# NethermindEth/latticefold

Hardware: AMD Instinct MI355X
Metric: folding-prover steps/sec (one NIFSProver::prove per step), GoldilocksRingNTT (higher is better)
Workload: dtype u64; 1 GPU; C4: GoldilocksRingNTT R1CS->CCS, m=N=2^20 rows, wit_len=262144, L=4, B=2^16, b=2, K=16, kappa=26, t=3; parallelism=replicas x1

## Files before the change

latticefold_amd/csrc/lf_capi.cpp:

```cpp
#include "lf_ring_host.h"
#include <thread>
#include <vector>

const char *lf_strerror(int code) {
    switch (code) {
        case LF_OK: return "ok";
        case LF_ERR_INVALID: return "invalid argument / wrong length";
        case LF_ERR_HIP: return "HIP runtime error (no GPU or out of device memory)";
        case LF_ERR_UNSUPPORTED: return "unsupported parameter";
        case LF_ERR_BAD_TABLES: return "ring tables are not a ring isomorphism";
        case LF_ERR_NORM: return "witness coefficient exceeds the decomposition bound";
        case LF_ERR_SIZE_BOUNDS: return "invalid size bounds (m must be >= wit_len*L, power of two)";
        case LF_ERR_STATE: return "call sequence misuse";
        case LF_ERR_REJECT: return "verifier rejected the proof";
    }
    return "unknown error";
}
const char *lf_phase_name(int i) { return (i >= 0 && i < LF_N_PHASES) ? PHASE_NAMES[i] : ""; }

static int install_tables(lf_ctx *c, u64 nonres, const u64 *y) {
    CrtTables T;
    if (build_crt_tables(nonres, y, T) != 0) return LF_ERR_BAD_TABLES;
    c->ring.T = T;
    c->dcrt = make_dev_crt(T);
    return ring_ops<GoldRing>::install_icrt(c, &T.icrt[0][0]);
}

int lf_ctx_create_ring(lf_ctx **out, int device, int ring) {
    if (ring == LF_RING_GOLDILOCKS) return lf_ctx_create(out, device);
    if (!out || ring != LF_RING_BABYBEAR) return LF_ERR_INVALID;
    lf_ctx *c = new lf_ctx();
    c->device = device;
    int rc = lfbb::BbCtx::create(&c->bb, c, device);
    if (rc != LF_OK) { delete c; return rc; }
    *out = c;
    return LF_OK;
}
int lf_ctx_device(const lf_ctx *c) { return c->device; }
int lf_ctx_ring(const lf_ctx *c) { return c && c->bb ? LF_RING_BABYBEAR : LF_RING_GOLDILOCKS; }
int lf_ring_words(int ring) { return ring == LF_RING_BABYBEAR ? 72 : (ring == LF_RING_GOLDILOCKS ? 24 : 0); }
int lf_ring_tau(int ring) { return ring == LF_RING_BABYBEAR ? 9 : (ring == LF_RING_GOLDILOCKS ? 3 : 0); }
uint64_t lf_ring_modulus(int ring) { return ring == LF_RING_BABYBEAR ? (uint64_t)lfbb::BB_P : (ring == LF_RING_GOLDILOCKS ? LF_P : 0); }

int lf_ctx_create(lf_ctx **out, int device) {
    if (!out) return LF_ERR_INVALID;
    int cnt = 0;
    if (hipGetDeviceCount(&cnt) != hipSuccess || cnt <= 0 || device < 0 || device >= cnt) return LF_ERR_HIP;
    HIPCHK(hipSetDevice(device));
    lf_ctx *c = new lf_ctx();
    c->device = device;
    int least = 0, greatest = 0;
    (void)hipDeviceGetStreamPriorityRange(&least, &greatest);
    if (c->create_lane_streams() != LF_OK || hipStreamCreateWithPriority(&c->st_io, hipStreamDefault, least) != hipSuccess) { delete c; return LF_ERR_HIP; }
    (void)hipEventCreateWithFlags(&c->ev_block, hipEventBlockingSync | hipEventDisableTiming);
    u64 nr, y[24];
    default_ring(&nr, y);
    int rc = install_tables(c, nr, y);
    if (rc != LF_OK) { delete c; return rc; }
    *out = c;
    return LF_OK;
}
static void planes_pool_drop(int device);
void lf_ctx_destroy(lf_ctx *c) {
    if (!c) return;
    while (c->io_jobs.load() > 0) std::this_thread::yield();
    (void)hipSetDevice(c->device);
    planes_pool_drop(c->device);
    if (c->bb) { c->bb->destroy(); delete c; return; }
    (void)c->sync_lanes();
    if (c->st_io) (void)hipStreamSynchronize(c->st_io);
    for (int l = 0; l < LF_NLANES; l++)
        if (c->stage[l]) (void)hipHostFree(c->stage[l]);
    if (c->h_pin2) { (void)hipHostFree(c->h_pin2); c->h_pin2 = nullptr; }
    if (c->ev_block) (void)hipEventDestroy(c->ev_block);
    c->comm[0].destroy();
    c->comm[1].destroy();
    if (c->tail_mail) (void)hipHostFree(c->tail_mail);
    if (c->tail_counters) (void)hipFree(c->tail_counters);
    if (c->d_poseidon) (void)hipFree(c->d_poseidon);
    if (c->ev_theta) (void)hipEventDestroy(c->ev_theta);
    if (c->ev_aux) (void)hipEventDestroy(c->ev_aux);
    if (c->st_aux) (void)hipStreamDestroy(c->st_aux);
    if (c->h_aux) (void)hipHostFree(c->h_aux);
    for (int i = 0; i < 2; i++)
        if (c->bits_ev[i]) (void)hipEventDestroy(c->bits_ev[i]);
    c->release_core();
    delete c;
}
int lf_set_ring_tables(lf_ctx *c, uint64_t nonres, const uint64_t *y) {
    if (!c || !y) return LF_ERR_INVALID;
    if (c->bb) return c->bb->set_ring_tables(nonres, y);
    std::lock_guard<std::mutex> g(c->mu);
    HIPCHK(hipSetDevice(c->device));
    return install_tables(c, nonres, y);
}
int lf_get_ring_tables(lf_ctx *c, uint64_t *nonres, uint64_t *y) {
    if (!c || !nonres || !y) return LF_ERR_INVALID;
    if (c->bb) return c->bb->get_ring_tables(nonres, y);
    *nonres = c->ring.T.nu;
    for (int k = 0; k < 8; k++)
        for (int q = 0; q < 3; q++) y[3 * k + q] = c->ring.T.y[k].c[q];
    return LF_OK;
}

int lf_set_digit_mode(lf_ctx *c, int mode) {
    if (!c || (mode != 0 && mode != 1)) return LF_ERR_INVALID;
    std::lock_guard<std::mutex> g(c->mu);
    c->core_any().digit_mode = mode;
    return LF_OK;
}
int lf_set_ext_basis(lf_ctx *c, const uint64_t *T) {
    if (!c || !T) return LF_ERR_INVALID;
    std::lock_guard<std::mutex> g(c->mu);
    const int ring = lf_ctx_ring(c);
    ExtBasis nb = c->xb;
    RET(nb.set(T, lf_ring_tau(ring), lf_ring_modulus(ring)));
    c->xb = nb;
    const int tt = nb.tau * nb.tau;
    if (c->bb) {
        lfbb::BbCtxImpl *b = c->bb->p;
        std::lock_guard<std::mutex> gb(b->mu);
        b->xb_on = nb.on;
        for (int i = 0; i < tt; i++) { b->xb_T[i] = lfbb::from_canon(nb.T[i]); b->xb_Ti[i] = lfbb::from_canon(nb.Ti[i]); }
    } else {
        c->xb_on = nb.on;
        for (int i = 0; i < tt; i++) { c->xb_T[i] = nb.T[i]; c->xb_Ti[i] = nb.Ti[i]; }
    }
    return LF_OK;
}
int lf_set_sharding(lf_ctx *c, int rank, int world, lf_exchange_fn cb, void *user) {
    if (!c || world < 1 || rank < 0 || rank >= world || (world & (world - 1)) != 0 || (world > 1 && !cb)) return LF_ERR_INVALID;
    if (c->bb) return c->bb->set_sharding(rank, world, cb, user);
// ... 983 lines not shown
```

latticefold_amd/csrc/lf_common.h:

```cpp
#pragma once
#include <hip/hip_runtime.h>

#include <stdlib.h>

#include <atomic>

#include "../../include/lfhip.h"

#define HIPCHK(x)                                    \
    do {                                             \
        hipError_t e__ = (x);                        \
        if (e__ != hipSuccess) return LF_ERR_HIP;    \
    } while (0)
#define RET(x)                      \
    do {                            \
        int rc__ = (x);             \
        if (rc__ != LF_OK) return rc__; \
    } while (0)

extern "C" void lfplus_scratch_trim(int device);
template <class T> static inline hipError_t lf_dev_malloc(T **p, size_t bytes) {
    hipError_t e = hipMalloc((void **)p, bytes);
    if (e != hipErrorOutOfMemory) return e;
    (void)hipGetLastError();
// ... 20 lines not shown
        bytes = want;
        return LF_OK;
    }
    void release() {
        if (p) (void)hipFree(p);
        p = nullptr;
        bytes = 0;
    }
};

inline uint64_t lf_next_witness_id() {
    static std::atomic<uint64_t> next{1};
    return next.fetch_add(1, std::memory_order_relaxed);
}
struct lf_witness {
    lf_ctx *ctx;
    int32_t *planes;
    size_t N;
    int device;
    size_t plane_bytes;
    uint64_t id = lf_next_witness_id();
    uint64_t *f_ntt = nullptr;
    size_t f_bytes = 0;
    uint64_t *w_ccs = nullptr;
    size_t w_bytes = 0;
};

int lf_planes_alloc(lf_ctx *ctx, size_t bytes, int32_t **out);
void lf_planes_release(lf_ctx *ctx, size_t bytes, int32_t *p);
int lf_ctx_device(const lf_ctx *ctx);


struct Tunables {
    bool lin_u_eval = false, fold_unfused = false, fold_no_lut = false, fold_tab_r1 = false, theta_eval = false, fold_no_r4tab = false, fold_no_r5tab = false;
    bool fold_rounds_no_split = false;
    bool fold_sv_no_split = false;
    bool lin_no_split = false;
    size_t lin_split_min = (size_t)1 << 17;
    bool no_live_rows = false;
    bool live_rows_low = false;
    size_t fold_split_min = 8192;
    bool force_exchange = false;
    bool device_transcript = false;
    bool shard_plain_rounds = false;
    int shard_two_lanes = -1;
    size_t shard_lin_min = 16384;
    size_t shard_fold_min = 2048;
    long i8_wgs = 0;
    bool lin_no_r1cs = false;
    bool lin_no_small = false;
    size_t dot_min = 4096;
    bool dot_valu = false;
    bool fold_witness_valu = false;
    bool fold_no_sv = false;
    size_t sv_min = 65536;
    int sv_rounds = 3;
    bool no_tail = false;
    size_t fuse_min = 16384, lut_min = (size_t)1 << 17, tab_min = 16384;
    size_t r5_min = 8192;
    size_t tail_n = 2048;
    static Tunables read(size_t lut_min_default) {
        Tunables t;
        t.lut_min = lut_min_default;
        const char *e;
        t.lin_u_eval = getenv("LF_LIN_U_EVAL") != nullptr;
        t.fold_unfused = getenv("LF_FOLD_UNFUSED") != nullptr;
        t.fold_no_lut = getenv("LF_FOLD_NO_LUT") != nullptr;
        t.fold_tab_r1 = getenv("LF_FOLD_TAB_R1") != nullptr;
        t.fold_no_r4tab = getenv("LF_FOLD_NO_R4TAB") != nullptr;
        t.fold_no_r5tab = getenv("LF_FOLD_NO_R5TAB") != nullptr;
        t.lin_no_split = getenv("LF_LIN_NO_SPLIT") != nullptr;
        t.fold_sv_no_split = getenv("LF_FOLD_SV_NO_SPLIT") != nullptr;
        t.no_live_rows = getenv("LF_NO_LIVE_ROWS") != nullptr;
        t.live_rows_low = getenv("LF_LIVE_ROWS_LOW") != nullptr;
        t.fold_rounds_no_split = getenv("LF_FOLD_ROUNDS_NO_SPLIT") != nullptr;
        if (const char *e = getenv("LF_LIN_SPLIT_MIN")) t.lin_split_min = (size_t)atoll(e);
        if (const char *e = getenv("LF_FOLD_SPLIT_MIN")) t.fold_split_min = (size_t)atoll(e);
        t.theta_eval = getenv("LF_THETA_EVAL") != nullptr;
        t.no_tail = getenv("LF_NO_TAIL") != nullptr;
        t.fold_no_sv = getenv("LF_FOLD_NO_SV") != nullptr;
        t.dot_valu = getenv("LF_DOT_VALU") != nullptr;
        t.fold_witness_valu = getenv("LF_FOLD_WITNESS_VALU") != nullptr;
        if ((e = getenv("LF_DOT_MIN"))) t.dot_min = (size_t)atoll(e);
        t.lin_no_small = getenv("LF_LIN_NO_SMALL") != nullptr;
        t.lin_no_r1cs = getenv("LF_LIN_NO_R1CS") != nullptr;
        if ((e = getenv("LF_FOLD_SV_MIN"))) t.sv_min = (size_t)atoll(e);
        if ((e = getenv("LF_FOLD_SV_ROUNDS"))) t.sv_rounds = atoi(e);
        if ((e = getenv("LF_I8_WGS"))) t.i8_wgs = atol(e);
        if ((e = getenv("LF_SHARD_TWO_LANES"))) t.shard_two_lanes = atoi(e) != 0;
        if ((e = getenv("LF_SHARD_LIN_MIN"))) t.shard_lin_min = (size_t)atoll(e);
        if ((e = getenv("LF_SHARD_FOLD_MIN"))) t.shard_fold_min = (size_t)atoll(e);
        t.shard_plain_rounds = getenv("LF_SHARD_PLAIN_ROUNDS") != nullptr;
        t.device_transcript = getenv("LF_DEVICE_TRANSCRIPT") != nullptr;
        t.force_exchange = getenv("LF_DIST_FORCE_EXCHANGE") != nullptr;
        if ((e = getenv("LF_FOLD_FUSE_MIN"))) t.fuse_min = (size_t)atoll(e);
        if ((e = getenv("LF_FOLD_LUT_MIN"))) t.lut_min = (size_t)atoll(e);
        if ((e = getenv("LF_FOLD_TAB_MIN"))) t.tab_min = (size_t)atoll(e);
        if ((e = getenv("LF_TAIL_N"))) t.tail_n = (size_t)atoll(e);
        if ((e = getenv("LF_FOLD_R5_MIN"))) t.r5_min = (size_t)atoll(e);
        return t;
    }
};

static inline int lf_validate_csr(unsigned t, size_t m, size_t n, const uint32_t *const *rowptr, const uint32_t *const *col,
                                  const uint64_t *const *val, int words, uint64_t modulus) {
    for (unsigned j = 0; j < t; j++) {
        if (!rowptr[j] || !col[j] || !val[j]) return LF_ERR_INVALID;
        if (rowptr[j][0] != 0) return LF_ERR_INVALID;
        for (size_t r = 0; r < m; r++)
            if (rowptr[j][r + 1] < rowptr[j][r]) return LF_ERR_INVALID;
        const size_t nnz = rowptr[j][m];
        for (size_t k = 0; k < nnz; k++)
            if (col[j][k] >= n) return LF_ERR_INVALID;
        for (size_t k = 0; k < nnz * (size_t)words; k++)
            if (val[j][k] >= modulus) return LF_ERR_INVALID;
    }
    return LF_OK;
}

struct ExtBasis {
    bool on = false;
    int tau = 0;
    uint64_t p = 0;
    uint64_t T[81], Ti[81];
    static uint64_t mulmod(uint64_t a, uint64_t b, uint64_t p) { return (uint64_t)(((unsigned __int128)a * b) % p); }
    void apply(const uint64_t *M, uint64_t *v) const {
        uint64_t o[9];
        for (int i = 0; i < tau; i++) {
            unsigned __int128 acc = 0;
            for (int j = 0; j < tau; j++) acc += (unsigned __int128)mulmod(M[i * tau + j], v[j], p);
            o[i] = (uint64_t)(acc % p);
        }
        for (int i = 0; i < tau; i++) v[i] = o[i];
    }
    void to_ext(uint64_t *v, size_t slots) const { if (on) for (size_t s = 0; s < slots; s++) apply(T, v + s * tau); }
// ... 34 lines not shown
```

latticefold_amd/csrc/lf_ctx.h:

```cpp
#pragma once
#include <hip/hip_runtime.h>
#include <assert.h>
#include <string.h>

#include <atomic>
#include <chrono>
#include <condition_variable>
#include <functional>
#include <future>
#include <thread>
#include <map>
#include <memory>
#include <mutex>
#include <set>
#include <string>
#include <vector>

#include "../../include/lfhip.h"
#include "bb_capi.h"
#include "lf_ctx_core.h"
#include "lf_common.h"
#include "lf_dist.h"
#include "lf_kernels.h"
#include "lf_live_rows.h"
// ... 74 lines not shown
        std::unique_lock<std::mutex> lk(m);
        for (;;) {
            cv.wait(lk, [&] { return has_job || stop; });
            if (stop) return;
            std::function<int()> j = std::move(job);
            has_job = false;
            lk.unlock();
            int r = j();
            lk.lock();
            rc = r;
            done = true;
            cv.notify_all();
        }
    }
    void submit(std::function<int()> j) {
        std::unique_lock<std::mutex> lk(m);
        if (!th.joinable()) th = std::thread([this] { loop(); });
        job = std::move(j);
        has_job = true;
        done = false;
        cv.notify_all();
    }
    int wait() {
        std::unique_lock<std::mutex> lk(m);
        cv.wait(lk, [&] { return done; });
        return rc;
    }
    ~LaneWorker() {
        {
            std::unique_lock<std::mutex> lk(m);
            stop = true;
            cv.notify_all();
        }
        if (th.joinable()) th.join();
    }
};

struct lf_ctx : CtxCore<u64> {
    lf_ctx() : CtxCore<u64>(8192, 2 * 9 * 24 * sizeof(u64)) {}
    int lane() const override { return t_lane; }
    lfbb::BbCtx *bb = nullptr;
    ExtBasis xb;
    hipStream_t &st_io = st_lane[2];
    std::mutex io_mu;
    std::atomic<int> io_jobs{0};
    inline CtxCoreBase &core_any();
    bool have_ccs_any() { return core_any().have_ccs; }
    const lf_params &params_any() { return core_any().P; }
    size_t n_any() { return core_any().n; }
    size_t m_any() { return core_any().m; }
    size_t N_any() { return core_any().N; }
    HostRing ring;
    DevCrt dcrt;
    LaneWorker lane1;
    int agreed_two_lanes = -1;
    bool two_lanes_ok = false;
    lfdist::Comm comm[2];
    lfdist::Comm &cm() { assert(t_lane < 2); return comm[t_lane]; }
    bool ccs_general = false;
    size_t live_rows = 0;
    lflive::Plan live_plan() const {
        if (tn.no_live_rows || sh_world > 1) return lflive::plan(m, m, 0, 0);
        return tn.live_rows_low ? lflive::plan(m, live_rows, lflive::GRANULE_LOW, lflive::MIN_M_LOW) : lflive::plan(m, live_rows, lflive::GRANULE, lflive::MIN_M);
    }
    size_t shc_r0 = (size_t)-1, shc_rcnt = 0, shc_lo = 0, shc_hi = 0;
    LinCombDesc desc{};
    std::vector<std::pair<const char *, double>> tl_marks;
    const lf_witness *bits_wit[2] = {nullptr, nullptr};
    u32 *bits_ptr[2] = {nullptr, nullptr};
    hipEvent_t bits_ev[2] = {nullptr, nullptr};
    hipEvent_t ev_yR = nullptr, ev_yL = nullptr;
    u64 *h_pin2 = nullptr;
    size_t h_pin2_words = 0;
    int pin2(size_t words) {
        if (words <= h_pin2_words) return LF_OK;
        if (h_pin2) (void)hipHostFree(h_pin2);
        h_pin2 = nullptr; h_pin2_words = 0;
        if (hipHostMalloc((void **)&h_pin2, words * 8) != hipSuccess) return LF_ERR_HIP;
        h_pin2_words = words;
        return LF_OK;
    }
    hipStream_t st_aux = nullptr;
    hipEvent_t ev_aux = nullptr;
    u64 *h_aux = nullptr;
    unsigned lin_split_rounds = 0;
    unsigned lin_live_rounds = 0;

    unsigned char *stage[LF_NLANES] = {nullptr, nullptr, nullptr};
    size_t stage_off[LF_NLANES] = {0, 0, 0};
    static constexpr size_t STAGE_BYTES = (size_t)1 << 20;
    int h2d_small(void *dst, const void *src, size_t bytes) {
        unsigned char *&ring = stage[t_lane];
        if (!ring && hipHostMalloc((void **)&ring, STAGE_BYTES, hipHostMallocDefault) != hipSuccess) { ring = nullptr; return LF_ERR_HIP; }
        const size_t need = (bytes + 63) & ~(size_t)63;
        if (need > STAGE_BYTES) {
            HIPCHK(hipMemcpyAsync(dst, src, bytes, hipMemcpyHostToDevice, stream()));
            HIPCHK(hipStreamSynchronize(stream()));
            return LF_OK;
        }
        if (stage_off[t_lane] + need > STAGE_BYTES) {
            HIPCHK(hipStreamSynchronize(stream()));
            stage_off[t_lane] = 0;
        }
        unsigned char *slot = ring + stage_off[t_lane];
        stage_off[t_lane] += need;
        memcpy(slot, src, bytes);
// ... 159 lines not shown
```

latticefold_amd/csrc/lf_kernels.h:

```cpp
#pragma once
#include "lf_ajtai_i8.h"
#include "lf_sv_rounds.h"
#include <hip/hip_runtime.h>

#include "lf_host.h"

namespace lf {

struct DevCrt {
    u64 nu;
    int nu2p40;
    u64 w4, w2, w10, w1, w7, w5, w11;
    int slot_of_pos[8], pos1[8], pos2[8];
    u64 tw1[8], tw2[8];
};
DevCrt make_dev_crt(const CrtTables &T);

struct Fq3Const { u64 c[3]; };

struct XbMat3 { u64 m[9]; };
void launch_aos_to_soa(const u64 *aos, u64 *soa, size_t n, hipStream_t s, u32 *flag = nullptr, const XbMat3 *Ti = nullptr);
void launch_soa_to_aos(const u64 *soa, u64 *aos, size_t n, hipStream_t s, const u32 *unless_flag = nullptr, const XbMat3 *T = nullptr);
void launch_ext_to_aos(const u64 *soa, u64 *aos, size_t n, hipStream_t s, const XbMat3 *T = nullptr);
void launch_slot_const_check(const u64 *tab, size_t n, u32 *flag, hipStream_t s);
void launch_fill_uniform(u64 *dst, size_t words, u64 seed, size_t start, hipStream_t s);
void launch_fill_ajtai(u64 *A, u32 kappa, size_t n, size_t n_total, size_t col0, u64 seed, hipStream_t s, u32 row0 = 0);

void launch_modsum(const u64 *parts, u32 nparts, size_t words, u64 *out, hipStream_t s);
void launch_gather_relayout(const u64 *all, u32 nranks, size_t planes, size_t lcl, u64 *full, hipStream_t s);
void launch_gather_relayout_part(const u64 *all, u32 nranks, size_t planes_tot, size_t p0, size_t planes, size_t lcl, u64 *full, hipStream_t s);

constexpr u32 SELFTEST_OUT = 13, SELFTEST_OUTC = 12;
void launch_selftest_field(const u64 *in, u32 n, u32 nc, u64 nu_gen, u64 *out, u64 *outc, u64 *mism_dev, hipStream_t s);

void launch_crt_fwd(const DevCrt &t, const u64 *coef, u64 *ntt, size_t n, hipStream_t s);
void launch_icrt_dense(const u64 *icrt_mat , const u64 *ntt, u64 *coef, size_t n, hipStream_t s);
void launch_ring_mul_ntt(const DevCrt &t, const u64 *a, const u64 *b, size_t n_terms, size_t n, u64 *out, hipStream_t s, u32 *flag = nullptr, const XbMat3 *Ti = nullptr);
void launch_ring_mul_coeff(const DevCrt &t, const u64 *icrt_mat , const u64 *a, const u64 *b, size_t n_terms, size_t n, u64 *out, hipStream_t s);


void launch_decompose(const u64 *coef, size_t n, u64 base, u32 digits, int layout, u64 *out, hipStream_t s, int mode = 0);
void launch_recompose(const u64 *in, size_t n_out, u64 base, u32 digits, u64 *out, hipStream_t s);
void launch_coef_to_i32(const u64 *coef, int32_t *planes, size_t n, u32 bound, int *viol, hipStream_t s);
void launch_i32_to_coef(const int32_t *planes, u64 *coef, size_t n, hipStream_t s);
void launch_recompose_crt(const DevCrt &t, const int32_t *planes, size_t n_planes, u32 wit_len, u32 L, u64 B, u32 K,
                          int mode_bits, u64 *out, size_t ldz, size_t off, hipStream_t s);
void launch_linf(const u64 *coef, size_t n, u64 *out_max, hipStream_t s);


void launch_build_eq(const DevCrt &t, const Fq3Const *r_dev , u32 nv, u64 *eq , hipStream_t s);
size_t build_eq_scratch_words(u32 nv);
void launch_build_eq2(const DevCrt &t, const Fq3Const *r_dev, u32 nv, u64 *scratch, u64 *eq, hipStream_t s);
void launch_spmv(const DevCrt &t, const u32 *rowptr, const u32 *col, const u64 *val , const u64 *z,
                 size_t ldz, u64 *out, size_t m, int accumulate, hipStream_t s, size_t r0 = 0, size_t rcnt = (size_t)-1 );
void launch_spmv_sum(const DevCrt &t, u32 nm, const u32 *const *rowptr, const u32 *const *col, const u64 *const *val, const u64 *z,
                     size_t z_stride, size_t ldz, u64 *out, size_t m, hipStream_t s, size_t r0 = 0, size_t rcnt = (size_t)-1 );
void launch_spmv_rows(const DevCrt &t, u32 nm, const u32 *const *rowptr, const u32 *const *col, const u64 *const *val, const u64 *z, size_t z_stride, size_t n,
                      u64 *zaos, u64 *out, size_t m, int accumulate, hipStream_t s, size_t r0 = 0, size_t rcnt = (size_t)-1);
void launch_spmv_t_eq(const DevCrt &t, const u32 *colptr, const u32 *rowidx, const u64 *val, const u64 *eq, size_t m,
                      u64 *q, size_t n, hipStream_t s, size_t c0 = 0, size_t ccnt = (size_t)-1 );
void launch_dot_batch(const DevCrt &t, const u64 *X, size_t ldx, u32 na, const u64 *Y, size_t ldy, u32 nb, size_t n,
                      u64 *partial, u64 *out, hipStream_t s);
size_t dot_partial_words(u32 na, u32 nb);
void launch_dot_eq(const DevCrt &t, const u64 *X, size_t ldx, u32 na, const u64 *eq, size_t ldeq, size_t n, u64 *partial,
                   u64 *out, hipStream_t s);
void launch_coef_eval(const DevCrt &t, const int32_t *planes, size_t n, const u64 *eq, size_t ldeq, u32 K, int mode_bits,
                      u64 *partial, u64 *out, hipStream_t s, size_t ldp = 0);
size_t coef_eval_partial_words(u32 K);
void launch_lincomb_z(const DevCrt &t, const u64 *z, size_t ldz, u32 K, const Fq3Const *coef_dev , u32 tt, size_t n,
                      u64 *out, hipStream_t s, u32 per_slot = 0);
void launch_add_fhat_comb(const DevCrt &t, const int32_t *planes, size_t n_planes, u32 K, const Fq3Const *apow_dev ,
                          u64 *G, size_t m, hipStream_t s, size_t r0 = 0, size_t rcnt = (size_t)-1 );
void launch_g_rows(const DevCrt &t, u32 nm, const u32 *const *rowptr, const u32 *const *col, const u64 *const *val, const u64 *z, size_t z_stride, size_t ldz, size_t live,
                   const int32_t *planes, size_t n_planes, u32 K, const Fq3Const *apow_dev , u64 *G, size_t m, hipStream_t s);

void launch_fix_ring(const DevCrt &t, const u64 *in, u64 *out, size_t n_in, Fq3Const r, hipStream_t s);
void launch_fix_fq3(const DevCrt &t, const u64 *in, u64 *out, size_t n_in, Fq3Const r, hipStream_t s);
size_t dot_i8_yb_bytes(size_t n);
size_t dot_i8_part_words(size_t n);
size_t dot_i8_tot_words();
int launch_dot_batch_i8(const DevCrt &t, const u64 *X, size_t ldx, u32 na, const u64 *Y, size_t ldy, u32 nb, size_t n, unsigned char *YB, int32_t *part,
                        long long *tot, u64 *out, hipStream_t s, bool y_packed = false, u32 nb_out = 0, u32 b0 = 0);
int launch_dot_pack_y(const u64 *X, const u64 *Y, size_t ldy, u32 nb, size_t n, unsigned char *YB, hipStream_t s);
void launch_vs_combine(const u64 *vs , u32 K, u64 *v , hipStream_t s);
void launch_fix_final(const DevCrt &t, const u64 *in , u32 rows3, Fq3Const r, u64 *out , hipStream_t s);

struct LinCombDesc {
    u32 t, q;
    u32 S_off[9];
    u32 S_idx[16];
    u64 c[8][24];
    int c_unit[8];
    u32 first[8];
    u32 ms[8];
};
void launch_lin_round(const DevCrt &t, const LinCombDesc &desc, const u64 *mz, size_t ld, const u64 *eq, size_t ldeq, size_t n,
                      u32 deg, u64 *partial, u64 *out, hipStream_t s, u32 max_blocks = 0, u32 split_xmask = 0 );
void launch_lin_round_fused(const DevCrt &t, const LinCombDesc &desc, const u64 *mz_prev, size_t ld_prev, const u64 *eq_prev, size_t ldeq_prev, Fq3Const r, u64 *mz_out,
                            size_t ld_out, u64 *eq_out, size_t ldeq_out, size_t n, u32 deg, u64 *partial, u64 *out, hipStream_t s, u32 max_blocks = 0,
// ... 106 lines not shown
```

latticefold_amd/csrc/lf_kernels.hip:

```cpp
#include "lf_kernels.h"

#include <stdlib.h>

#include "lf_kernels_dev.cuh"
#include "lf_sb.h"

namespace lf {


DevCrt make_dev_crt(const CrtTables &T) {
    DevCrt d;
    d.nu = T.nu; d.nu2p40 = T.nu_is_2p40;
    d.w4 = T.w4; d.w2 = T.w2; d.w10 = T.w10; d.w1 = T.w1; d.w7 = T.w7; d.w5 = T.w5; d.w11 = T.w11;
    for (int p = 0; p < 8; p++) {
        d.slot_of_pos[p] = T.slot_of_pos[p]; d.pos1[p] = T.pos1[p]; d.pos2[p] = T.pos2[p];
        d.tw1[p] = T.tw1[p]; d.tw2[p] = T.tw2[p];
    }
    return d;
}


__global__ void __launch_bounds__(256) k_modsum(const u64 *parts, u32 nparts, size_t words, u64 *out) {
    size_t w = (size_t)blockIdx.x * 256 + threadIdx.x;
    if (w >= words) return;
// ... 127 lines not shown
            int32_t v = planes[(size_t)c * n_planes + i * L + l];
            if (mode_bits) {
                int d = digit2(v, k);
                if (d > 0) acc = fq_add(acc, bp.v[l]);
                else if (d < 0) acc = fq_sub(acc, bp.v[l]);
            } else {
                u64 mag = (u64)(v < 0 ? -v : v);
                u64 term = fq_mul(bp.v[l], mag);
                acc = v < 0 ? fq_sub(acc, term) : fq_add(acc, term);
            }
        }
        a[c] = acc;
    }
    crt_store(a, out + (size_t)k * 24 * ldz, ldz, off + i, t);
}
struct BInt4 { long long v[4]; };
__global__ void __launch_bounds__(256) k_recompose_crt_b4(DevCrt t, const int32_t *planes, size_t n_planes, u32 wit_len, BInt4 bi, u32 K,
                                                           u64 *out, size_t ldz, size_t off) {
    size_t i = (size_t)blockIdx.x * 256 + threadIdx.x;
    const u32 u = blockIdx.y;
    if (i >= wit_len) return;
    const size_t jj = off + i;
    int4 w[8];
#pragma unroll
    for (int v8 = 0; v8 < 8; v8++) w[v8] = *(const int4 *)(planes + (size_t)(3 * v8 + u) * n_planes + 4 * i);
    int plane[8];
    u64 tw[8];
#pragma unroll
    for (int p = 0; p < 8; p++) {
        int s3 = 3 * t.slot_of_pos[p];
        plane[p] = u == 0 ? s3 : (u == 1 ? s3 + t.pos1[p] : s3 + t.pos2[p]);
        tw[p] = u == 1 ? t.tw1[p] : t.tw2[p];
    }
    for (u32 k = 0; k < K; k++) {
        u64 x[8], A[8];
#pragma unroll
        for (int v8 = 0; v8 < 8; v8++) {
            const int32_t v[4] = {w[v8].x, w[v8].y, w[v8].z, w[v8].w};
            long long sacc = 0;
#pragma unroll
            for (int l = 0; l < 4; l++) {
                int d = digit2(v[l], k);
                sacc += d > 0 ? bi.v[l] : (d < 0 ? -bi.v[l] : 0ll);
            }
            x[v8] = sacc < 0 ? LF_P - (u64)(-sacc) : (u64)sacc;
        }
        lfk::crt8<GoldF>(x, A, t);
        u64 *o = out + (size_t)k * 24 * ldz;
#pragma unroll
        for (int p = 0; p < 8; p++) o[(size_t)plane[p] * ldz + jj] = u == 0 ? A[p] : fq_mul(tw[p], A[p]);
    }
}
void launch_recompose_crt(const DevCrt &t, const int32_t *planes, size_t n_planes, u32 wit_len, u32 L, u64 B, u32 K, int mode_bits,
                          u64 *out, size_t ldz, size_t off, hipStream_t s) {
    if (mode_bits && L == 4 && B < ((u64)1 << 20) && (n_planes & 3) == 0 && ((uintptr_t)planes & 15) == 0) {
        BInt4 bi;
        bi.v[0] = 1;
        for (int l = 1; l < 4; l++) bi.v[l] = bi.v[l - 1] * (long long)B;
        hipLaunchKernelGGL(k_recompose_crt_b4, dim3(cdiv(wit_len, 256), 3), dim3(256), 0, s, t, planes, n_planes, wit_len, bi, K, out, ldz, off);
        return;
    }
    BPow bp;
    u64 pw = 1;
    for (int l = 0; l < 8; l++) { bp.v[l] = pw; pw = fq_mul(pw, B % LF_P); }
    hipLaunchKernelGGL(k_recompose_crt, dim3(cdiv(wit_len, 256), K), dim3(256), 0, s, t, planes, n_planes, wit_len, L, bp, K, mode_bits,
                       out, ldz, off);
}
__global__ void __launch_bounds__(256) k_sb_recompose_crt(DevCrt t, const unsigned char *D, size_t ldn, u32 wit_len, u32 L, BPow bp, u64 *out, size_t ldz, size_t off) {
    size_t i = (size_t)blockIdx.x * 256 + threadIdx.x;
    u32 k = blockIdx.y;
    if (i >= wit_len) return;
    u64 a[24];
#pragma unroll
    for (int c = 0; c < 24; c++) {
        u64 acc = 0;
        for (u32 l = 0; l < L; l++) {
            const int d = (int)D[((size_t)k * 24 + c) * ldn + i * L + l] - 64;
            const u64 term = fq_mul(bp.v[l], (u64)(d < 0 ? -d : d));
            acc = d < 0 ? fq_sub(acc, term) : fq_add(acc, term);
        }
        a[c] = acc;
    }
    crt_store(a, out + (size_t)k * 24 * ldz, ldz, off + i, t);
}
int launch_sb_recompose_crt(const DevCrt &t, const unsigned char *D, size_t ldn, u32 wit_len, u32 L, u64 B, u32 K, u64 *out, size_t ldz, size_t off, hipStream_t s) {
    if (!wit_len || L > 8) return -1;
    BPow bp;
    u64 pw = 1;
    for (int l = 0; l < 8; l++) { bp.v[l] = pw; pw = fq_mul(pw, B % LF_P); }
    hipLaunchKernelGGL(k_sb_recompose_crt, dim3(cdiv(wit_len, 256), K), dim3(256), 0, s, t, D, ldn, wit_len, L, bp, out, ldz, off);
    return hipGetLastError() == hipSuccess ? 0 : -1;
}


struct Acc5 { AccP s[5]; };
__device__ __forceinline__ void acc5_zero(Acc5 &a) {
#pragma unroll
    for (int i = 0; i < 5; i++) accp_zero(a.s[i]);
}
__device__ __forceinline__ void acc5_mac(Acc5 &a, const u64 x[3], const u64 y[3]) {
    accp_mad(a.s[0], x[0], y[0]);
    accp_mad(a.s[1], x[0], y[1]); accp_mad(a.s[1], x[1], y[0]);
    accp_mad(a.s[2], x[0], y[2]); accp_mad(a.s[2], x[1], y[1]); accp_mad(a.s[2], x[2], y[0]);
    accp_mad(a.s[3], x[1], y[2]); accp_mad(a.s[3], x[2], y[1]);
    accp_mad(a.s[4], x[2], y[2]);
}
template <bool NU>
__device__ __forceinline__ Fq3 acc5_finish(const Acc5 &a, u64 nu) {
// ... 602 lines not shown
```

latticefold_amd/csrc/lf_prove.cpp:

```cpp
#include "lf_ring_host.h"


static int run_lin_sumcheck(lf_ctx *c, Transcript &tr, const u64 *mz, const u64 *eqb, u64 *msgs , Fq3 *point, u64 *u_dev = nullptr,
                            const std::function<void(u32)> *after_round = nullptr, const Fq3 *beta = nullptr, size_t live = 0) {
    const lf_params &P = c->P;
    u32 deg = P.d + 1;
    size_t m = c->m;
    u64 *fx[2], *fe[2], *partial, *od;
    RET(c->tbuf("lin_fix0", (size_t)P.t * 24 * (m / 2), &fx[0]));
    RET(c->tbuf("lin_fix1", (size_t)P.t * 24 * (m / 4 ? m / 4 : 1), &fx[1]));
    RET(c->tbuf("lin_efix0", 3 * (m / 2), &fe[0]));
    RET(c->tbuf("lin_efix1", 3 * (m / 4 ? m / 4 : 1), &fe[1]));
    RET(c->tbuf("round_partial", round_partial_words(), &partial));
    od = c->round_out();
    if (!od) return LF_ERR_HIP;
    { HostTimer ht(c); lfs::sumcheck_prologue<GoldV>(tr, P.s, deg); }
    const u64 *cur = mz, *cure = eqb;
    size_t n = m;
    int flip = 0;
    size_t nl = live && live < m && c->sh_world == 1 ? live : m;
    const size_t Gw = (size_t)c->sh_world, gr = (size_t)c->sh_rank;
    bool sharded = shard_keep(c, 0, m);
    u64 *od_dev = nullptr;
    if (Gw > 1) RET(c->tbuf("lin_round_out", (size_t)(deg + 1) * 24 + 8, &od_dev));
// ... 69 lines not shown
            if (round == 1) cure = fe[0];
            else if (nl < n) launch_eq_pairsum(preve + nl, prevn / 2, (n - nl) / 2, (u64 *)cure + nl / 2, n / 2, c->stream());
        } else if (fused_now) {
            launch_lin_round_fused(c->dcrt, c->desc, prev, prevn, preve, prevn, f3c(point[round - 2]), (u64 *)cur, n, (u64 *)cure, n, nl, deg, partial, od, c->stream(), c->lin_blocks);
            if (nl < n) launch_fix_many(c->dcrt, preve + 2 * nl, prevn, (u64 *)cure + nl, n, prevn - 2 * nl, 1, f3c(point[round - 2]), c->stream());
        }
        else launch_lin_round(c->dcrt, c->desc, cur, n, cure, n, nl, deg, partial, od, c->stream(), c->lin_blocks);
        RET(c->lane_sync());
        if (split) {
            HostTimer ht2(c);
            c->lin_split_rounds++;
            lfs::complete_lin_split(hv, sp, dT, od, round >= 2 ? msgs + (size_t)(round - 2) * (deg + 1) * 24 : nullptr, point[round >= 2 ? round - 2 : 0], ev);
        } else
        memcpy(ev, od, (size_t)(deg + 1) * 24 * 8);
        HostTimer ht(c);
        point[round - 1] = lfs::sumcheck_round<GoldV>(tr, ev, deg + 1);
        if (after_round) (*after_round)(round);
        if (round <= 2 || round == 4 || round == 8) TL_MARK_ROUND("  lin round", round);
    }
    TL_MARK("  lin rounds done");
    if (u_dev) launch_fix_final(c->dcrt, cur, P.t * 8, f3c(point[P.s - 1]), u_dev, c->stream());
    return LF_OK;
}

int shard_col_range(lf_ctx *c, size_t r0, size_t rcnt, size_t *lo, size_t *hi) {
    static std::mutex mu;
    std::lock_guard<std::mutex> g(mu);
    if (c->shc_r0 != r0 || c->shc_rcnt != rcnt) {
        size_t mn = c->n, mx = 0;
        std::vector<u32> rp(2), cl;
        for (u32 j = 0; j < c->P.t; j++) {
            HIPCHK(hipMemcpy(&rp[0], c->d_rowptr[j] + r0, 4, hipMemcpyDeviceToHost));
            HIPCHK(hipMemcpy(&rp[1], c->d_rowptr[j] + r0 + rcnt, 4, hipMemcpyDeviceToHost));
            if (rp[1] <= rp[0]) continue;
            cl.resize(rp[1] - rp[0]);
            HIPCHK(hipMemcpy(cl.data(), c->d_col[j] + rp[0], cl.size() * 4, hipMemcpyDeviceToHost));
            for (u32 v : cl) { if (v < mn) mn = v; if ((size_t)v + 1 > mx) mx = (size_t)v + 1; }
        }
        if (mx <= mn) { mn = 0; mx = 0; }
        c->shc_r0 = r0; c->shc_rcnt = rcnt; c->shc_lo = mn; c->shc_hi = mx;
    }
    *lo = c->shc_lo; *hi = c->shc_hi;
    return LF_OK;
}
int build_z(lf_ctx *c, const int32_t *planes, u32 K, int mode_bits, const u64 *heads , u64 *z ,
            size_t w0, size_t wcnt, const unsigned char *D) {
    const lf_params &P = c->P;
    u32 hl = P.l + 1;
    if (wcnt == (size_t)-1) { w0 = 0; wcnt = P.wit_len; }
    if (D) {
        if (w0 != 0 || wcnt != P.wit_len || !mode_bits) return LF_ERR_UNSUPPORTED;
        if (launch_sb_recompose_crt(c->dcrt, D, sb_ld(c->N), P.wit_len, P.L, P.B, K, z, c->n, hl, c->stream()) != 0) return LF_ERR_HIP;
    } else
    if (wcnt) launch_recompose_crt(c->dcrt, planes + w0 * P.L, c->N, (u32)wcnt, P.L, P.B, K, mode_bits, z, c->n, hl + w0, c->stream());
    std::vector<u64> h((size_t)K * 24 * hl);
    for (u32 k = 0; k < K; k++)
        for (u32 i = 0; i < hl; i++)
            for (int w = 0; w < 24; w++) h[((size_t)k * 24 + w) * hl + i] = heads[((size_t)k * hl + i) * 24 + w];
    u64 *stage;
    RET(c->tbuf("z_heads", h.size(), &stage));
    RET(c->h2d_small(stage, h.data(), h.size() * 8));
    HIPCHK(hipMemcpy2DAsync(z, c->n * 8, stage, hl * 8, hl * 8, (size_t)K * 24, hipMemcpyDeviceToDevice, c->stream()));
    return LF_OK;
}

static int linearize_impl(lf_ctx *c, Transcript &tr, const u64 *cccs, const lf_witness *wit, u64 *lcccs_out, u64 *proof, u64 **eq_r_keep) {
    const lf_params &P = c->P;
    size_t m = c->m, n = c->n;
    size_t ph = c->ev_begin(10);
    std::vector<u64> head((size_t)(P.l + 1) * 24);
    memcpy(head.data(), cccs + (size_t)P.kappa * 24, (size_t)P.l * 24 * 8);
    HostRing::from_u64(1, head.data() + (size_t)P.l * 24);
    u64 *z, *mz, *eqb, *eqr, *partial, *od;
    RET(c->tbuf("lin_z", 24 * n, &z));
    RET(c->tbuf("lin_mz", (size_t)P.t * 24 * m, &mz));
    RET(c->tbuf("lin_eqb", 3 * m, &eqb));
    RET(c->tbuf("eq_r_R", 3 * m, &eqr));
    RET(c->tbuf("red_partial", 256 * 4096, &partial));
    RET(c->tbuf("lin_small", 4096, &od));
    RET(build_z(c, wit->planes, 1, 0, head.data(), z));
    TL_MARK("  lin z enqueued");
    std::vector<Fq3> beta(P.s);
    {
        HostTimer ht(c);
        tr.absorb_label("beta_s");
        for (u32 i = 0; i < P.s; i++) beta[i] = tr.get_challenge();
    }
    RET(build_eq_dev(c, beta.data(), P.s, eqb));
    const size_t live = c->tn.lin_u_eval ? m : c->live_plan().pad;
    {
        const size_t Gw = (size_t)c->sh_world;
        const bool rows_sliced = shard_keep(c, 0, m) && !c->tn.lin_u_eval;
        const size_t r0 = rows_sliced ? (size_t)c->sh_rank * (m / Gw) : 0, rcnt = rows_sliced ? m / Gw : live;
        if (c->ccs_general) {
            u64 *zaos;
            RET(c->tbuf("spmv_zaos", (size_t)P.t * n * 24, &zaos));
            launch_soa_to_aos(z, zaos, n, c->stream());
            for (u32 j = 0; j < P.t; j++)
                launch_spmv_rows(c->dcrt, 1, &c->d_rowptr[j], &c->d_col[j], &c->d_val[j], nullptr, 0, n, zaos, mz + (size_t)j * 24 * m, m, 0, c->stream(), r0, rcnt);
        } else
        for (u32 j = 0; j < P.t; j++)
            launch_spmv(c->dcrt, c->d_rowptr[j], c->d_col[j], c->d_val[j], z, n, mz + (size_t)j * 24 * m, m, 0, c->stream(), r0, rcnt);
    }
    std::vector<Fq3> pt(P.s);
    const bool u_eval = c->tn.lin_u_eval;
    TL_MARK("  lin Mz enqueued");
    struct VsSplit {
// ... 580 lines not shown
```

Measured before the change: 64.47 steps/s.

## Recompose CRT witness bits via int8 MFMA matrix multiply

Adds an int8 MFMA kernel for recomposing bit-decomposed witness planes into CRT-form z columns. The ring-map matrix is precomputed once as signed byte limbs, with a bias, by probing the existing kernel with unit vectors. Each bit slice then becomes a 32x32x32 i8 matrix product plus carry reassembly, replacing the VALU 64-bit modular arithmetic path. It adds a cached per-context table and a host sync during preparation, and falls back to the old kernel when the table structure check fails.

```diff
diff --git a/latticefold_amd/csrc/lf_capi.cpp b/latticefold_amd/csrc/lf_capi.cpp
--- a/latticefold_amd/csrc/lf_capi.cpp
+++ b/latticefold_amd/csrc/lf_capi.cpp
@@ -23,6 +23,7 @@
     if (build_crt_tables(nonres, y, T) != 0) return LF_ERR_BAD_TABLES;
     c->ring.T = T;
     c->dcrt = make_dev_crt(T);
+    c->zk_i8.state = 0;
     return ring_ops<GoldRing>::install_icrt(c, &T.icrt[0][0]);
 }
 
@@ -78,6 +79,7 @@
     if (c->tail_mail) (void)hipHostFree(c->tail_mail);
     if (c->tail_counters) (void)hipFree(c->tail_counters);
     if (c->d_poseidon) (void)hipFree(c->d_poseidon);
+    if (c->zk_i8.dev) (void)hipFree(c->zk_i8.dev);
     if (c->ev_theta) (void)hipEventDestroy(c->ev_theta);
     if (c->ev_aux) (void)hipEventDestroy(c->ev_aux);
     if (c->st_aux) (void)hipStreamDestroy(c->st_aux);
diff --git a/latticefold_amd/csrc/lf_common.h b/latticefold_amd/csrc/lf_common.h
--- a/latticefold_amd/csrc/lf_common.h
+++ b/latticefold_amd/csrc/lf_common.h
@@ -96,6 +96,7 @@
     size_t dot_min = 4096;
     bool dot_valu = false;
     bool fold_witness_valu = false;
+    bool zk_valu = false;
     bool fold_no_sv = false;
     size_t sv_min = 65536;
     int sv_rounds = 3;
@@ -125,6 +126,7 @@
         t.fold_no_sv = getenv("LF_FOLD_NO_SV") != nullptr;
         t.dot_valu = getenv("LF_DOT_VALU") != nullptr;
         t.fold_witness_valu = getenv("LF_FOLD_WITNESS_VALU") != nullptr;
+        t.zk_valu = getenv("LF_ZK_VALU") != nullptr;
         if ((e = getenv("LF_DOT_MIN"))) t.dot_min = (size_t)atoll(e);
         t.lin_no_small = getenv("LF_LIN_NO_SMALL") != nullptr;
         t.lin_no_r1cs = getenv("LF_LIN_NO_R1CS") != nullptr;
diff --git a/latticefold_amd/csrc/lf_ctx.h b/latticefold_amd/csrc/lf_ctx.h
--- a/latticefold_amd/csrc/lf_ctx.h
+++ b/latticefold_amd/csrc/lf_ctx.h
@@ -150,6 +150,15 @@
     size_t N_any() { return core_any().N; }
     HostRing ring;
     DevCrt dcrt;
+    ZkI8 zk_i8;
+    std::mutex zk_mu;
+    int zk_i8_get(u64 B, const ZkI8 **out) {
+        std::lock_guard<std::mutex> g(zk_mu);
+        if (zk_i8.state == 0 || zk_i8.B != B)
+            if (zk_i8_prepare(dcrt, B, &zk_i8, stream()) != 0) return LF_ERR_HIP;
+        *out = zk_i8.state == 1 ? &zk_i8 : nullptr;
+        return LF_OK;
+    }
     LaneWorker lane1;
     int agreed_two_lanes = -1;
     bool two_lanes_ok = false;
diff --git a/latticefold_amd/csrc/lf_kernels.h b/latticefold_amd/csrc/lf_kernels.h
--- a/latticefold_amd/csrc/lf_kernels.h
+++ b/latticefold_amd/csrc/lf_kernels.h
@@ -43,8 +43,16 @@
 void launch_recompose(const u64 *in, size_t n_out, u64 base, u32 digits, u64 *out, hipStream_t s);
 void launch_coef_to_i32(const u64 *coef, int32_t *planes, size_t n, u32 bound, int *viol, hipStream_t s);
 void launch_i32_to_coef(const int32_t *planes, u64 *coef, size_t n, hipStream_t s);
+struct ZkI8;
 void launch_recompose_crt(const DevCrt &t, const int32_t *planes, size_t n_planes, u32 wit_len, u32 L, u64 B, u32 K,
-                          int mode_bits, u64 *out, size_t ldz, size_t off, hipStream_t s);
+                          int mode_bits, u64 *out, size_t ldz, size_t off, hipStream_t s, const ZkI8 *zk = nullptr);
+struct ZkI8 {
+    u64 B = 0;
+    int state = 0;
+    int *dev = nullptr;
+};
+int zk_i8_prepare(const DevCrt &t, u64 B, ZkI8 *zk, hipStream_t s);
+int launch_recompose_crt_i8(const ZkI8 &zk, const int32_t *planes, size_t n_planes, u32 wit_len, u32 K, u64 *out, size_t ldz, size_t off, hipStream_t s);
 void launch_linf(const u64 *coef, size_t n, u64 *out_max, hipStream_t s);
 
 
diff --git a/latticefold_amd/csrc/lf_kernels.hip b/latticefold_amd/csrc/lf_kernels.hip
--- a/latticefold_amd/csrc/lf_kernels.hip
+++ b/latticefold_amd/csrc/lf_kernels.hip
@@ -203,8 +203,9 @@
     }
 }
 void launch_recompose_crt(const DevCrt &t, const int32_t *planes, size_t n_planes, u32 wit_len, u32 L, u64 B, u32 K, int mode_bits,
-                          u64 *out, size_t ldz, size_t off, hipStream_t s) {
+                          u64 *out, size_t ldz, size_t off, hipStream_t s, const ZkI8 *zk) {
     if (mode_bits && L == 4 && B < ((u64)1 << 20) && (n_planes & 3) == 0 && ((uintptr_t)planes & 15) == 0) {
+        if (zk && zk->state == 1 && zk->B == B && launch_recompose_crt_i8(*zk, planes, n_planes, wit_len, K, out, ldz, off, s) != 1) return;
         BInt4 bi;
         bi.v[0] = 1;
         for (int l = 1; l < 4; l++) bi.v[l] = bi.v[l - 1] * (long long)B;
diff --git a/latticefold_amd/csrc/lf_prove.cpp b/latticefold_amd/csrc/lf_prove.cpp
--- a/latticefold_amd/csrc/lf_prove.cpp
+++ b/latticefold_amd/csrc/lf_prove.cpp
@@ -145,7 +145,11 @@
         if (w0 != 0 || wcnt != P.wit_len || !mode_bits) return LF_ERR_UNSUPPORTED;
         if (launch_sb_recompose_crt(c->dcrt, D, sb_ld(c->N), P.wit_len, P.L, P.B, K, z, c->n, hl, c->stream()) != 0) return LF_ERR_HIP;
     } else
-    if (wcnt) launch_recompose_crt(c->dcrt, planes + w0 * P.L, c->N, (u32)wcnt, P.L, P.B, K, mode_bits, z, c->n, hl + w0, c->stream());
+    if (wcnt) {
+        const ZkI8 *zk = nullptr;
+        if (mode_bits && !c->tn.zk_valu && c->sh_world == 1 && P.L == 4 && P.B < ((u64)1 << 20)) RET(c->zk_i8_get(P.B, &zk));
+        launch_recompose_crt(c->dcrt, planes + w0 * P.L, c->N, (u32)wcnt, P.L, P.B, K, mode_bits, z, c->n, hl + w0, c->stream(), zk);
+    }
     std::vector<u64> h((size_t)K * 24 * hl);
     for (u32 k = 0; k < K; k++)
         for (u32 i = 0; i < hl; i++)
diff --git a/latticefold_amd/csrc/lf_zk_i8.hip b/latticefold_amd/csrc/lf_zk_i8.hip
--- /dev/null
+++ b/latticefold_amd/csrc/lf_zk_i8.hip
@@ -0,0 +1,145 @@
+#include <hip/hip_runtime.h>
+
+#include <vector>
+
+#include "lf_common.h"
+#include "lf_field.cuh"
+#include "lf_kernels.h"
+
+namespace lf {
+typedef int v4i __attribute__((ext_vector_type(4)));
+typedef int v16i __attribute__((ext_vector_type(16)));
+
+constexpr size_t ZK_A_WORDS = 3 * 2 * 64 * 4;
+constexpr size_t ZK_TAB_WORDS = ZK_A_WORDS + 24 + 3;
+
+typedef unsigned short zk_us2 __attribute__((ext_vector_type(2)));
+__device__ __forceinline__ int zk_digits(u32 mag, u32 sgn, u32 kk) {
+    const u32 t = (mag >> kk) & 0x01010101u;
+    const zk_us2 m = __builtin_bit_cast(zk_us2, t) * zk_us2{255, 255};
+    return (int)(__builtin_bit_cast(u32, m) & sgn);
+}
+
+__global__ void __launch_bounds__(256) __attribute__((amdgpu_waves_per_eu(4, 4))) k_recompose_crt_i8(const int *tab, const int32_t *planes, size_t n_planes, u32 wit_len, u32 K, u64 *out, size_t ldz, size_t off) {
+    const u32 lane = threadIdx.x & 63, wave = threadIdx.x >> 6, nn = lane & 31, h = lane >> 5, u = blockIdx.y;
+    const size_t i0 = ((size_t)blockIdx.x * 4 + wave) * 32;
+    if (i0 >= wit_len) return;
+    const size_t i = i0 + nn;
+    const bool live = i < wit_len;
+    const size_t li = live ? i : 0;
+    const v4i a0 = *(const v4i *)(tab + ((u * 2 + 0) * 64 + lane) * 4), a1 = *(const v4i *)(tab + ((u * 2 + 1) * 64 + lane) * 4);
+    size_t orow[4];
+#pragma unroll
+    for (int j = 0; j < 4; j++) orow[j] = (size_t)tab[ZK_A_WORDS + 8 * u + 2 * j + h] * ldz + off + i;
+    const u32 bX = (u32)tab[ZK_A_WORDS + 24], bY = (u32)tab[ZK_A_WORDS + 25], bZ = (u32)tab[ZK_A_WORDS + 26];
+    int4 w[4];
+#pragma unroll
+    for (int jj = 0; jj < 4; jj++) w[jj] = *(const int4 *)(planes + (size_t)(u + 3 * (4 * h + jj)) * n_planes + 4 * li);
+    u32 sgn[4];
+#pragma unroll
+    for (int jj = 0; jj < 4; jj++)
+        sgn[jj] = (w[jj].x < 0 ? 0xFFu : 1u) | (w[jj].y < 0 ? 0xFF00u : 0x100u) | (w[jj].z < 0 ? 0xFF0000u : 0x10000u) | (w[jj].w < 0 ? 0xFF000000u : 0x1000000u);
+    for (u32 kb = 0; kb < K; kb += 8) {
+        u32 mag[4];
+#pragma unroll
+        for (int jj = 0; jj < 4; jj++) {
+            const u32 m0 = (u32)(w[jj].x < 0 ? -w[jj].x : w[jj].x), m1 = (u32)(w[jj].y < 0 ? -w[jj].y : w[jj].y), m2 = (u32)(w[jj].z < 0 ? -w[jj].z : w[jj].z),
+                      m3 = (u32)(w[jj].w < 0 ? -w[jj].w : w[jj].w);
+            mag[jj] = ((m0 >> kb) & 0xFFu) | (((m1 >> kb) & 0xFFu) << 8) | (((m2 >> kb) & 0xFFu) << 16) | (((m3 >> kb) & 0xFFu) << 24);
+        }
+#pragma unroll
+        for (u32 kk = 0; kk < 8; kk++) {
+            if (kb + kk >= K) break;
+            const v4i b = v4i{zk_digits(mag[0], sgn[0], kk), zk_digits(mag[1], sgn[1], kk), zk_digits(mag[2], sgn[2], kk), zk_digits(mag[3], sgn[3], kk)};
+            const v16i zero = {0, 0, 0, 0, 0, 0, 0, 0, 0, 0, 0, 0, 0, 0, 0, 0};
+            const v16i c0 = __builtin_amdgcn_mfma_i32_32x32x32_i8(a0, b, zero, 0, 0, 0), c1 = __builtin_amdgcn_mfma_i32_32x32x32_i8(a1, b, zero, 0, 0, 0);
+            u64 *o = out + (size_t)(kb + kk) * 24 * ldz;
+#pragma unroll
+            for (int j = 0; j < 4; j++) {
+                const u32 X = (u32)(c0[4 * j] + 256 * c0[4 * j + 1] + 65536 * c0[4 * j + 2]) + bX;
+                const u32 Y = (u32)(c0[4 * j + 3] + 256 * c1[4 * j] + 65536 * c1[4 * j + 1]) + bY;
+                const u32 Z = (u32)(c1[4 * j + 2] + 256 * c1[4 * j + 3]) + bZ;
+                const u64 T = (u64)Y + ((u64)Z << 24);
+                const u64 lo = (T << 24) + X;
+                const u64 hi = (T >> 40) + (lo < X);
+                if (live) o[orow[j]] = fq_canon(fq_reduce128_loose(lo, hi));
+            }
+            __builtin_amdgcn_sched_barrier(0);
+        }
+    }
+}
+
+int zk_i8_prepare(const DevCrt &t, u64 B, ZkI8 *zk, hipStream_t s) {
+    zk->state = 0;
+    zk->B = B;
+    std::vector<int32_t> hp((size_t)24 * 384, 0);
+    for (int c = 0; c < 24; c++)
+        for (int l = 0; l < 4; l++) hp[(size_t)c * 384 + (size_t)(4 * c + l) * 4 + l] = 1;
+    std::vector<u64> U((size_t)24 * 96);
+    void *scratch = nullptr;
+    const size_t pb = hp.size() * 4, ub = U.size() * 8;
+    if (!zk->dev && lf_dev_malloc(&zk->dev, ZK_TAB_WORDS * 4) != hipSuccess) return -1;
+    if (lf_dev_malloc(&scratch, pb + ub) != hipSuccess) return -1;
+    int32_t *dp = (int32_t *)scratch;
+    u64 *du = (u64 *)((char *)scratch + pb);
+    bool ok = hipMemcpyAsync(dp, hp.data(), pb, hipMemcpyHostToDevice, s) == hipSuccess;
+    if (ok) {
+        launch_recompose_crt(t, dp, 384, 96, 4, B, 1, 0, du, 96, 0, s);
+        ok = hipGetLastError() == hipSuccess && hipMemcpyAsync(U.data(), du, ub, hipMemcpyDeviceToHost, s) == hipSuccess && hipStreamSynchronize(s) == hipSuccess;
+    }
+    (void)hipFree(scratch);
+    if (!ok) return -1;
+    std::vector<int> tab(ZK_TAB_WORDS, 0);
+    int cnt[3] = {0, 0, 0}, pl[3][8];
+    for (int w = 0; w < 24; w++) {
+        int cls = -1;
+        for (int e = 0; e < 96; e++) {
+            U[(size_t)w * 96 + e] = fq_canon(U[(size_t)w * 96 + e]);
+            if (U[(size_t)w * 96 + e] == 0) continue;
+            const int ue = (e / 4) % 3;
+            if (cls >= 0 && cls != ue) { zk->state = -1; return 0; }
+            cls = ue;
+        }
+        if (cls < 0 || cnt[cls] == 8) { zk->state = -1; return 0; }
+        pl[cls][cnt[cls]++] = w;
+    }
+    for (int u = 0; u < 3; u++)
+        for (int p = 0; p < 8; p++) tab[ZK_A_WORDS + 8 * u + p] = pl[u][p];
+    for (int u = 0; u < 3; u++)
+        for (int p = 0; p < 8; p++)
+            for (int q = 0; q < 8; q++)
+                for (int l = 0; l < 4; l++) {
+                    const u64 T = U[(size_t)pl[u][p] * 96 + 4 * (u + 3 * q) + l];
+                    __int128 v = T > 0x7F7F7F7F7F7F7F7Full ? (__int128)T - (__int128)LF_P : (__int128)T;
+                    for (int byte = 0; byte < 8; byte++) {
+                        const int d = (int)(int8_t)(unsigned char)(v & 0xFF);
+                        v = (v - d) / 256;
+                        const int tl = byte >> 2, m = 8 * (p >> 1) + 4 * (p & 1) + (byte & 3), ln = 32 * (q >> 2) + m;
+                        tab[((size_t)(u * 2 + tl) * 64 + ln) * 4 + (q & 3)] |= (int)(((u32)d & 0xFFu) << (8 * l));
+                    }
+                    if (v != 0) { zk->state = -1; return 0; }
+                }
+    {
+        __int128 N = (__int128)17 * (__int128)LF_P - (__int128)4096 * (__int128)0x0101010101010101ull;
+        u32 beta[8];
+        for (int b = 0; b < 8; b++) {
+            const u32 nb = b < 7 ? (u32)(N & 0xFF) : (u32)N;
+            beta[b] = 4096 + nb;
+            N >>= 8;
+        }
+        if (beta[7] >= 4096 + 256) { zk->state = -1; return 0; }
+        tab[ZK_A_WORDS + 24] = (int)(beta[0] + 256 * beta[1] + 65536 * beta[2]);
+        tab[ZK_A_WORDS + 25] = (int)(beta[3] + 256 * beta[4] + 65536 * beta[5]);
+        tab[ZK_A_WORDS + 26] = (int)(beta[6] + 256 * beta[7]);
+    }
+    if (hipMemcpyAsync(zk->dev, tab.data(), tab.size() * 4, hipMemcpyHostToDevice, s) != hipSuccess || hipStreamSynchronize(s) != hipSuccess) return -1;
+    zk->state = 1;
+    return 0;
+}
+
+int launch_recompose_crt_i8(const ZkI8 &zk, const int32_t *planes, size_t n_planes, u32 wit_len, u32 K, u64 *out, size_t ldz, size_t off, hipStream_t s) {
+    if (zk.state != 1 || !zk.dev || wit_len == 0 || K < 1 || K > 32 || (n_planes & 3) || ((uintptr_t)planes & 15) || ((uintptr_t)out & 7)) return 1;
+    hipLaunchKernelGGL(k_recompose_crt_i8, dim3((wit_len + 127) / 128, 3), dim3(256), 0, s, (const int *)zk.dev, planes, n_planes, wit_len, K, out, ldz, off);
+    return hipGetLastError() == hipSuccess ? 0 : -1;
+}
+}
```

Result: faster. 65.28 steps/s (median of 6 runs) (+1.2%).
